# ns1labs/pktvisor

Hardware: AMD Instinct MI355X
Metric: Mpkt/s device-resident (Net+DNS handler parse) (higher is better)
Workload: dtype u8; 1 GPU; C2: Net+DNS handlers, 64 B UDP (Eth+IPv4+UDP+22 B), Zipf IPs, host_spec 10.x.x.x/8; records_per_gpu=10000000, handlers=net v1 + dns v1 (default groups), parallelism=dp1

## Files before the change

### pktvisor_amd/csrc/pv_kernels.hip

```cpp
#include <cstring>
#include <hip/hip_runtime.h>
#include <rocprim/rocprim.hpp>
#include <stdint.h>

#include "pv_layout.h"
#include "pv_geodb.h"

#define PV_BLOCK 256
#define PV_C __attribute__((address_space(4)))
#ifdef PV_STAMPS
#define STAMP_DECL                                                                           \
    uint64_t st_acc[8] = {0, 0, 0, 0, 0, 0, 0, 0};                                          \
    uint64_t st_prev = __builtin_amdgcn_s_memtime();
#define STAMP(k)                                                                             \
    {                                                                                        \
        const uint64_t now = __builtin_amdgcn_s_memtime();                                   \
        st_acc[k] += now - st_prev;                                                          \
        st_prev = now;                                                                       \
    }
#define STAMP_FLUSH                                                                          \
    if ((threadIdx.x & 63) == 0)                                                             \
        for (int k_ = 0; k_ < 8; k_++) P.stamps[((uint64_t)blockIdx.x * (blockDim.x / 64) + threadIdx.x / 64) * 8 + k_] = st_acc[k_];
#else
#define STAMP_DECL
// ... 1628 lines not shown
            const uint64_t m = __ballot(isdns);
            if (m) {
                uint32_t q = 0;
                if (lane == 0) q = atomicAdd(&S.nd, (uint32_t)__popcll(m));
                q = __builtin_amdgcn_readlane(q, 0);
                const uint32_t below = __builtin_amdgcn_mbcnt_hi((uint32_t)(m >> 32), __builtin_amdgcn_mbcnt_lo((uint32_t)m, 0u));
                if (isdns) {
                    PV_G uint4 *dd = reinterpret_cast<PV_G uint4 *>(K.dq) + 2 * (dq_base + q + below);
                    dd[0] = dm.a;
                    dd[1] = dm.b;
                }
            }
            if (tops && i <= r1 && !(K.dbg & 128)) K.iplog[i] = ek;
            if (K.tcp_emit) {
                const uint64_t tm = __ballot(istcp);
                if (tm) {
                    if (lane == 0) K.tmask[t] = tm;
                    tcp_seg_store(K.tseg, K.tseg_cnt, K.tseg_cap, hasseg, seg, lane);
                }
            }
        }
        STAMP(6)
        return released;
    };
    for (uint32_t k = 0; k < ntl; k++) {
        PV_VMCNT((PV_NL_Q - 1) * PV_NL_OPS);
        STAMP(1)
        const uint32_t sl = k % PV_NL_Q, row = k % PV_NL_OROWS;
        const bool rel = tile_body(k, NW.lo[row][lane], __builtin_amdgcn_readfirstlane(NW.lo[row][0]),
                                   tile_of(k) * PV_WT + PV_WT >= n ? (uint32_t)K.rec_bytes : __builtin_amdgcn_readfirstlane(NW.hi[row]),
                                   NW.slot[sl]);
        if (!rel) refill(k);
    }
    PV_VMCNT(0);
    if (wslot != 0xffffffffu) knet_flush(K, wslot, c);
    __syncthreads();
    for (uint32_t b = threadIdx.x; b < PV_HBINS; b += blockDim.x)
        if (S.hist[b]) ksum_add(K, hslot, PV_OFF_PAYLOAD + b, S.hist[b]);
    STAMP_FLUSH
    if (threadIdx.x == 0) {
        P.mq_cnt[blockIdx.x] = 0;
        P.dq_cnt[blockIdx.x] = S.nd;
        if (S.nd) atomicAdd(P.n_dns, S.nd);
    }
}



struct FastRec {
    uint32_t ok, caplen, dir, l4, syn, l4len;
};
struct HostNets {
    uint32_t a0, m0, a1, m1, e0, e1;
};
PV_FN uint32_t hit4(const HostNets &h, uint32_t ip)
{
    const uint32_t m = (((ip ^ h.a0) & h.m0) == 0 ? h.e0 : 0u) | (((ip ^ h.a1) & h.m1) == 0 ? h.e1 : 0u);
    return ip ? m : 0u;
}
PV_FN FastRec fast_fields(const RecW &r, const HostNets &h)
{
    FastRec f;
    f.caplen = r.w[2];
    const uint32_t w3 = r.w[7], w4 = r.w[8], w5 = r.w[9];
    const uint32_t proto = w5 >> 24;
    f.ok = (f.caplen >= 34) & ((w3 & 0xffffffu) == 0x450008u) & (proto != 4) & (proto != 41);
    const uint32_t total = ((w4 & 0xff) << 8) | ((w4 >> 8) & 0xff);
    const uint32_t frag = ((w5 & 0xff) << 8) | ((w5 >> 8) & 0xff);
    const uint32_t l = f.caplen - 14;
    const uint32_t len = (total != 0 && total < l) ? total : l;
    const uint32_t pll = len - 20;
    const bool l4ok = (len > 20) & !(frag & 0x3fff);
    const bool udp = l4ok & (proto == 17) & (pll >= 8);
    const bool tcp = l4ok & (proto == 6) & (pll >= 20);
    f.l4 = udp ? 17u : (tcp ? 6u : 0u);
    f.syn = tcp ? (r.w[15] >> 25) & 1 : 0u;
    f.l4len = pll;
    const uint32_t dst = hit4(h, r.at(46)), src = hit4(h, r.at(42));
    f.dir = dst ? 0u : (src ? 1u : 2u);
    return f;
}
PV_FN uint32_t dns_port_bf(uint32_t pw)
{
    const uint32_t sport = ((pw & 0xff) << 8) | ((pw >> 8) & 0xff);
    const uint32_t dport = ((pw >> 8) & 0xff00) | (pw >> 24);
    const bool dd = (dport == 53) | (dport == 5353) | (dport == 5355) | (dport == 53000);
    const bool sd = (sport == 53) | (sport == 5353) | (sport == 5355) | (sport == 53000);
    return dd ? sport : (sd ? dport : 0u);
}
PV_FN Parsed fast_parsed(const FastRec &f, const RecW &r, uint32_t ts_nano, uint64_t off)
{
    Parsed o;
    o.caplen = f.caplen;
    o.sec = r.w[0];
    o.nsec = ts_nano ? (int32_t)r.w[1] : (int32_t)(r.w[1] * 1000u);
    o.frame = off + 16;
    o.l3 = 4; o.l4 = (uint8_t)f.l4; o.has4 = 1; o.has6 = 0; o.syn = (uint8_t)f.syn; o.dir = (uint8_t)f.dir;
    o.v4 = o.frame + 14; o.v6 = 0;
    o.l4off = f.l4 ? o.frame + 34 : 0;
    o.l4len = f.l4 ? f.l4len : 0;
    return o;
}
__device__ __forceinline__ SlowOut net_slow_p(const PvParams *__restrict__ Pp, const SAcc R, uint64_t off, uint64_t i)
{
    PV_CREF(PvParams) P = *(const PV_C PvParams *)Pp;
    NetK K;
    K.recs = P.recs; K.offs = P.offs; K.n = P.n; K.rec_bytes = P.rec_bytes; K.gbase = P.gbase;
    K.sum = P.sum; K.cpc = P.cpc; K.iplog = P.iplog; K.dq = P.dq; K.flags = P.flags;
    K.n_shift = 0; K.skip_before = 0; K.slot0 = P.slot_of[0];
    K.net_groups = P.net_groups; K.dbg = 0; K.net_filter_all = 0;
    K.n_dshift = P.n_dshift; K.dskip_before = P.dskip_before;
    K.tcp_emit = P.tcp_emit; K.tseg_cap = P.tseg_cap; K.tseg = P.tseg; K.tseg_cnt = P.tseg_cnt; K.tmask = P.tmask;
    K.ndeep_net = nullptr; K.ndeep_dns = nullptr; K.gfilt = nullptr;
    return net_slow_body(R, parse_cfg(P), P, K, off, i, K.slot0, true);
}

#ifndef PV_REG_MINW
#define PV_REG_MINW 2
#endif
struct NetRegState {
    uint32_t hist[PV_HBINS];
    uint32_t nd, nx, ns;
    int64_t dord[PV_MAX_SHIFTS];
};
__device__ __forceinline__ void win_load(const PV_G uint8_t *recs, uint32_t off, uint4 (&W)[5])
{
    const PV_G uint4 *p = reinterpret_cast<const PV_G uint4 *>(recs + (off & ~3u));
#pragma unroll
    for (int j = 0; j < 5; j++) W[j] = p[j];
}
__device__ __forceinline__ void win_words(const uint4 (&W)[5], uint32_t sh, RecW &r)
{
    uint32_t x[17];
#pragma unroll
    for (int k = 0; k < 4; k++) { x[4 * k] = W[k].x; x[4 * k + 1] = W[k].y; x[4 * k + 2] = W[k].z; x[4 * k + 3] = W[k].w; }
    x[16] = W[4].x;
#pragma unroll
    for (int j = 0; j < 16; j++) r.w[j] = __builtin_amdgcn_alignbyte(x[j + 1], x[j], sh);
}
#ifdef PV_TSTAMPS
#define PV_TST_NET ((1u << 20) + (1u << 18))
#define TST_WALL(P, k) if (threadIdx.x == 0) (P).stamps[PV_TST_NET + 4ull * blockIdx.x + (k)] = wall_clock64();
#define TST_WALL_XCC(P) \
    if (threadIdx.x == 0) (P).stamps[PV_TST_NET + 4ull * blockIdx.x] = (wall_clock64() & ~(0xfull << 60)) | (uint64_t)__builtin_amdgcn_s_getreg(20 | (3 << 11)) << 60;
#else
#define TST_WALL_XCC(P)
#define TST_WALL(P, k)
#endif
__device__ __forceinline__ void net_ranges(PV_CREF(PvParams) P, bool contig, uint32_t &lb0, uint32_t &lb1, uint32_t &step)
{
    lb0 = blockIdx.x; lb1 = P.grid_main; step = gridDim.x;
    if (contig) { lb0 = min(blockIdx.x * P.cb_fan, P.grid_main); lb1 = min(lb0 + P.cb_fan, P.grid_main); step = 1; }
}
struct FuseRing {
    struct Sec {
        uint32_t ip[PV_RING_SLOTS][PV_WT];
        uint64_t dm[PV_RING_SLOTS];
    } sec[2];
};
template <uint32_t NW, bool TC = false, bool FUSE = false, bool RING = false>
__device__ __forceinline__ void net_fast_reg(const PvParams *__restrict__ Pp, FuseRing *ring = nullptr)
{
    static_assert(!RING || (FUSE && TC && NW == PV_RING_WAVES), "the ring is the fused kernel's");
    PV_CREF(PvParams) P = *(const PV_C PvParams *)Pp;
    __shared__ NetRegState S;
    TST_WALL_XCC(P)
    const uint32_t wave = __builtin_amdgcn_readfirstlane(threadIdx.x >> 6), lane = threadIdx.x & 63;
    for (uint32_t b = threadIdx.x; b < PV_HBINS; b += (FUSE ? 64u * NW : blockDim.x)) S.hist[b] = 0;
    if (threadIdx.x == 0) { S.nd = 0; S.nx = 0; S.ns = 0; }
    if (threadIdx.x < PV_MAX_SHIFTS) S.dord[threadIdx.x] = P.dpos[threadIdx.x];
    __syncthreads();
    const PV_G uint8_t *const recs = P.recs;
    const bool compact = P.ip_compact;
    const PV_G uint32_t *const offs = P.offs;
    const uint64_t n = P.n, last = n - 1;
    const uint32_t slot = P.slot_of[0];
    const uint32_t groups = P.net_groups;
    const bool tops = groups & PV_NET_TOP_IPS_BIT, card = groups & PV_NET_CARDINALITY_BIT;
    const uint32_t ts_nano = P.ts_nano;
    HostNets h;
    {
        const uint32_t n4 = P.nets.n4;
        h.a0 = P.nets.v4_addr[0]; h.m0 = P.nets.v4_mask[0]; h.e0 = n4 > 0 ? ~0u : 0u;
        h.a1 = P.nets.v4_addr[1]; h.m1 = P.nets.v4_mask[1]; h.e1 = n4 > 1 ? ~0u : 0u;
    }
    const uint64_t nwt = (n + PV_WT - 1) / PV_WT;
    uint64_t cd = 0, cl = 0;
    NetCtr c;
    c.zero();
    bool any = false;
    uint32_t secn = 0;
#ifdef PV_RANGE_AB
    uint32_t lb0, lb1, lbstep;
    net_ranges(P, FUSE || P.net_contig, lb0, lb1, lbstep);
    for (uint32_t lb = lb0; lb < lb1; lb += lbstep) {
#else
    for (uint32_t lb = FUSE ? blockIdx.x * P.cb_fan : blockIdx.x; lb < (FUSE ? min(blockIdx.x * P.cb_fan + P.cb_fan, P.grid_main) : P.grid_main);
         lb += FUSE ? 1u : gridDim.x) {
#endif
    const uint64_t wbeg = (uint64_t)lb * P.wt_per_block;
    const uint64_t wend = min<uint64_t>(wbeg + P.wt_per_block, nwt);
    const uint32_t ntl = wend > wbeg + wave ? (uint32_t)((wend - wbeg - wave + NW - 1) / NW) : 0u;
    any |= ntl != 0;
    const uint32_t nsk = RING ? pv_ring_sections(wend > wbeg ? (uint32_t)(wend - wbeg) : 0u) * PV_RING_K : 0u;
    auto tile_of = [&](uint32_t k) -> uint64_t { return wbeg + wave + (uint64_t)NW * min(k, RING && !ntl ? 0u : ntl - 1); };
    auto off_of = [&](uint32_t k) -> uint32_t { return offs[min<uint64_t>(tile_of(k) * PV_WT + lane, last)]; };
    PV_G uint64_t *const trash = P.trash + ((uint64_t)blockIdx.x * NW + wave) * 256;
    auto tile = [&](uint32_t k, uint32_t off, const uint4 (&W)[5]) {
        const bool live = k < ntl;
        const uint64_t t = tile_of(k);
        const uint64_t r0 = t * PV_WT, i = r0 + lane;
        const bool active = live && i < n;
        RecW rw;
        win_words(W, off & 3, rw);
        const FastRec f = fast_fields(rw, h);
        const bool fast = active & (f.ok != 0);
        const uint64_t slowm = __ballot(active & !fast);
        cd += fast ? 1ull << (f.dir * 16) : 0ull;
        cl += fast ? (1ull << (f.l4 == 17 ? 0u : (f.l4 == 6 ? 16u : 32u))) + ((uint64_t)f.syn << 48) : 0ull;
        uint32_t hv = fast ? f.caplen : PV_NOH;
        const uint32_t ip = f.dir == 0 ? rw.at(42) : rw.at(46);
        const bool ipok = fast & (f.dir != 2) & (ip != 0);
        uint64_t ek = tops && ipok ? ((uint64_t)slot << 60) | ((uint64_t)TM_IPV4 << 56) | ((uint64_t)card << 33) |
                                         ((uint64_t)f.dir << 32) | ip
                                   : 0ull;
        if (card && !tops) {
            if (ipok) {
                uint64_t h1, h2;
                murmur_8((uint64_t)(int64_t)(int32_t)ip, h1, h2);
                __hip_atomic_fetch_min(P.cpc + (uint64_t)slot * PV_MIN_WORDS + (uint64_t)(f.dir == 0 ? CPC_SRC : CPC_DST) * PV_CPC_COUPONS +
                                           cpc_coupon(h1, h2),
                                       (int64_t)(P.gbase + i), __ATOMIC_RELAXED, __HIP_MEMORY_SCOPE_AGENT);
            }
        }
        const uint32_t port = (fast & (f.l4 == 17)) ? dns_port_bf(rw.at(50)) : 0u;
        DnsMsgW dm{};
        bool isdns = port != 0;
        if (__ballot(isdns)) {
            if (isdns) {
                const Parsed o = fast_parsed(f, rw, ts_nano, off);
                uint32_t dp = 0;
                for (uint32_t q = 0; q < P.n_dshift; q++) dp += (int64_t)(4 * i) >= S.dord[q];
                const SAcc R{recs, nullptr, 0, 0, 0, 1};
                DnsMsg d = dns_msg_of(P, R, o, i, port, dp, dp >= P.dskip_before, false);
                d.fkey = fast_flowkey(rw);
                dm = msg_words(d);
            }
        }
        bool istcp = fast & (f.l4 == 6), hasseg = false;
        PvTcpSeg seg;
        const uint32_t temit = P.tcp_emit;
        if (temit && __ballot(istcp)) {
            if (istcp) hasseg = tcp_seg_fast(rw, fast_parsed(f, rw, ts_nano, off), i, seg);
        }
        if (slowm) {
            uint32_t q = 0;
            if (lane == 0) q = atomicAdd(&S.ns, (uint32_t)__popcll(slowm));
            q = __builtin_amdgcn_readlane(q, 0) + __builtin_amdgcn_mbcnt_hi((uint32_t)(slowm >> 32), __builtin_amdgcn_mbcnt_lo((uint32_t)slowm, 0u));
            if (active && !fast) P.slow_list[wbeg * PV_WT + q] = (uint32_t)i;
        }
        if (__ballot(hv != PV_NOH && hv > 65535)) {
            if (hv != PV_NOH && hv > 65535) { atomicOr(P.flags, PVF_BIG_CAPLEN); hv = 65535; }
        }
        hist_add(S.hist, P.sum + (uint64_t)slot * PV_SUM_WORDS + PV_OFF_PAYLOAD, hv, lane);
        const uint64_t m = __ballot(isdns);
        if (m) {
            uint32_t q = 0;
            if (lane == 0) q = atomicAdd(&S.nd, (uint32_t)__popcll(m));
            q = __builtin_amdgcn_readlane(q, 0);
            const uint32_t below = __builtin_amdgcn_mbcnt_hi((uint32_t)(m >> 32), __builtin_amdgcn_mbcnt_lo((uint32_t)m, 0u));
            if (isdns) {
                PV_G uint4 *dd = reinterpret_cast<PV_G uint4 *>(P.dq) + 2 * (wbeg * PV_WT + q + below);
                dd[0] = dm.a;
                dd[1] = dm.b;
            }
        }
        if (TC || tops) {
            if (TC || compact) {
                const bool v4 = ek && ((ek >> 32) & ~1ull) == (P.ip_base >> 32);
                const uint64_t xm = __ballot(active && ek && !v4);
                const uint64_t dbit = __ballot(v4 && ((ek >> 32) & 1));
                if constexpr (RING) {
                    FuseRing::Sec &rs = ring->sec[secn & 1];
                    const uint32_t q = pv_ring_slot(wave, k);
                    rs.ip[q][lane] = active && v4 ? (uint32_t)ek : 0u;
                    if (lane == 0) rs.dm[q] = dbit;
                } else if (TC) {
#ifdef PV_FUSE_NOSTORE
                    if constexpr (!FUSE)
#endif
                    {
                    PV_G uint32_t *const l32 = live ? P.iplog32 + i : reinterpret_cast<PV_G uint32_t *>(trash) + lane;
                    PV_G uint64_t *const ldw = live ? P.ipdir + t : trash + 32;
                    *l32 = active && v4 ? (uint32_t)ek : 0u;
                    *ldw = dbit;
                    }
                } else if (live) {
                    if (active) P.iplog32[i] = v4 ? (uint32_t)ek : 0u;
                    if (lane == 0) P.ipdir[t] = dbit;
                }
                if (xm) {
                    uint32_t q = 0;
                    if (lane == 0) q = atomicAdd(&S.nx, (uint32_t)__popcll(xm));
                    q = __builtin_amdgcn_readlane(q, 0);
                    const uint32_t below = __builtin_amdgcn_mbcnt_hi((uint32_t)(xm >> 32), __builtin_amdgcn_mbcnt_lo((uint32_t)xm, 0u));
                    if (active && ek && !v4) {
                        P.iplog[wbeg * PV_WT + q + below] = ek;
                        P.ipx_rep[wbeg * PV_WT + q + below] = (uint32_t)i;
                    }
                }
            } else if (active) {
                P.iplog[i] = ek;
            }
        }
        if (temit) {
            const uint64_t tm = __ballot(istcp);
            if (tm) {
                if (lane == 0) P.tmask[t] = tm;
                tcp_seg_store(P.tseg, P.tseg_cnt, P.tseg_cap, hasseg, seg, lane);
            }
        }
    };
    static_assert(PV_RING_K == 3, "a section is one turn of the pipeline loop");
    if (RING ? nsk : ntl) {
        uint4 W0[5], W1[5], W2[5];
        uint32_t o0 = off_of(0), o1 = off_of(1), o2 = off_of(2);
        win_load(recs, o0, W0);
        win_load(recs, o1, W1);
        for (uint32_t k = 0; k < (RING ? nsk : ntl); k += 3) {
            const uint32_t oN = off_of(k + 3);
            win_load(recs, o2, W2);
            tile(k, o0, W0);
            const uint32_t oN1 = off_of(k + 4);
            win_load(recs, oN, W0);
            o0 = oN;
            tile(k + 1, o1, W1);
            const uint32_t oN2 = off_of(k + 5);
            win_load(recs, oN1, W1);
            o1 = oN1;
            tile(k + 2, o2, W2);
            o2 = oN2;
            if constexpr (RING) {
                lds_barrier();
                secn++;
            }
        }
    }
    if constexpr (FUSE && !RING) __builtin_amdgcn_s_waitcnt(PV_WAIT_VMCNT0);
    lds_barrier();
    if (threadIdx.x == 0) {
        P.mq_cnt[lb] = 0;
        P.dq_cnt[lb] = S.nd;
        if (compact) P.ipx_cnt[lb] = S.nx;
        P.slow_cnt[lb] = S.ns;
        if (S.nd) atomicAdd(P.n_dns, S.nd);
        if (S.ns) atomicAdd(P.n_slow, S.ns);
        S.nd = 0;
        S.nx = 0;
        S.ns = 0;
    }
    lds_barrier();
    }
    {
        const uint32_t fin = (uint32_t)(cd & 0xffff), fout = (uint32_t)((cd >> 16) & 0xffff), funk = (uint32_t)((cd >> 32) & 0xffff);
        const uint32_t nf = fin + fout + funk;
        c.nev += nf; c.n4 += nf;
        c.nin += fin; c.nout += fout; c.nunk += funk;
        c.nudp += (uint32_t)(cl & 0xffff); c.ntcp += (uint32_t)((cl >> 16) & 0xffff);
        c.noth += (uint32_t)((cl >> 32) & 0xffff); c.nsyn += (uint32_t)(cl >> 48);
    }
    NetK K;
    K.sum = P.sum; K.net_groups = groups; K.net_filter_all = 0; K.gfilt = nullptr;
    if (any) knet_flush(K, slot, c);
    lds_barrier();
    for (uint32_t b = threadIdx.x; b < PV_HBINS; b += (FUSE ? 64u * NW : blockDim.x))
        if (S.hist[b]) ksum_add(K, slot, PV_OFF_PAYLOAD + b, S.hist[b]);
    TST_WALL(P, 1)
}

#ifndef PV_SPAN_MAX
#define PV_SPAN_MAX 6144
#endif
typedef uint32_t v4u32 __attribute__((ext_vector_type(4)));
struct NetSpanState {
    uint32_t hist[PV_HBINS];
    uint32_t nd, ns;
    int64_t dord[PV_MAX_SHIFTS];
    v4u32 buf[4][PV_SPAN_MAX / 16 + 8];
};
struct SpanX {
    v4u32 v0, v1, v2, v3, v4, v5;
};
__device__ __forceinline__ void span_load(const PV_G uint8_t *recs, uint32_t o, uint32_t lane, SpanX &X, uint32_t &b)
{
    const uint32_t o0 = __builtin_amdgcn_readfirstlane(o), o63 = __builtin_amdgcn_readlane(o, 63);
    const uint32_t b16 = o0 & ~15u;
    const uint32_t len = o63 + 80u - b16;
    const PV_G v4u32 *ps = reinterpret_cast<const PV_G v4u32 *>(recs + b16);
    const bool sp = o63 >= o0 && len <= PV_SPAN_MAX && !__ballot(o < o0 || o > o63);
    b = sp ? b16 : 0xffffffffu;
    const uint32_t lim = sp ? len : 0u;
#define PV_SPAN_LD(j) X.v##j = ps[16u * (lane + 64u * j) < lim ? lane + 64u * j : 0u]
    PV_SPAN_LD(0); PV_SPAN_LD(1); PV_SPAN_LD(2); PV_SPAN_LD(3); PV_SPAN_LD(4); PV_SPAN_LD(5);
#undef PV_SPAN_LD
}
extern "C" __global__ void __launch_bounds__(256) __attribute__((amdgpu_waves_per_eu(PV_REG_MINW))) pv_net_kernel_span(const PvParams *__restrict__ Pp)
{
    PV_CREF(PvParams) P = *(const PV_C PvParams *)Pp;
    __shared__ NetSpanState S;
    constexpr uint32_t NW = 4;
    const uint32_t wave = __builtin_amdgcn_readfirstlane(threadIdx.x >> 6), lane = threadIdx.x & 63;
    for (uint32_t b = threadIdx.x; b < PV_HBINS; b += blockDim.x) S.hist[b] = 0;
    if (threadIdx.x == 0) { S.nd = 0; S.ns = 0; }
    if (threadIdx.x < PV_MAX_SHIFTS) S.dord[threadIdx.x] = P.dpos[threadIdx.x];
    __syncthreads();
    const PV_G uint8_t *const recs = P.recs;
    const PV_G uint32_t *const offs = P.offs;
    const uint64_t n = P.n, last = n - 1;
    const uint32_t slot = P.slot_of[0];
    const uint32_t groups = P.net_groups;
    const bool card = groups & PV_NET_CARDINALITY_BIT;
    const uint32_t ts_nano = P.ts_nano;
    HostNets h;
    {
        const uint32_t n4 = P.nets.n4;
        h.a0 = P.nets.v4_addr[0]; h.m0 = P.nets.v4_mask[0]; h.e0 = n4 > 0 ? ~0u : 0u;
        h.a1 = P.nets.v4_addr[1]; h.m1 = P.nets.v4_mask[1]; h.e1 = n4 > 1 ? ~0u : 0u;
    }
    const uint64_t nwt = (n + PV_WT - 1) / PV_WT;
    uint64_t cd = 0, cl = 0;
    v4u32 *Lq = S.buf[wave];
    for (uint32_t lb = blockIdx.x; lb < P.grid_main; lb += gridDim.x) {
    const uint64_t wbeg = (uint64_t)lb * P.wt_per_block;
    const uint64_t wend = min<uint64_t>(wbeg + P.wt_per_block, nwt);
    const uint32_t ntl = wend > wbeg + wave ? (uint32_t)((wend - wbeg - wave + NW - 1) / NW) : 0u;
    auto tile_of = [&](uint32_t k) -> uint64_t { return wbeg + wave + (uint64_t)NW * min(k, ntl - 1); };
    auto off_of = [&](uint32_t k) -> uint32_t { return offs[min<uint64_t>(tile_of(k) * PV_WT + lane, last)]; };
    auto tile = [&](uint32_t k, uint32_t off, const SpanX &X, uint32_t b) {
        const uint64_t t = tile_of(k);
        const uint64_t i = t * PV_WT + lane;
        const bool active = i < n;
        RecW rw;
        if (b != 0xffffffffu) {
            Lq[lane] = X.v0; Lq[lane + 64] = X.v1; Lq[lane + 128] = X.v2;
            Lq[lane + 192] = X.v3; Lq[lane + 256] = X.v4; Lq[lane + 320] = X.v5;
            asm volatile("" ::: "memory");
            const uint32_t rel = off - b;
            const v4u32 *q = Lq + (rel >> 4);
            uint32_t x[24];
#pragma unroll
            for (int j = 0; j < 6; j++) {
                const v4u32 v = q[j];
                x[4 * j] = v.x; x[4 * j + 1] = v.y; x[4 * j + 2] = v.z; x[4 * j + 3] = v.w;
            }
            uint32_t m1 = 0u - ((rel >> 2) & 1), m2 = 0u - ((rel >> 3) & 1);
            asm volatile("" : "+v"(m1), "+v"(m2));
            uint32_t y[19], z[17];
#pragma unroll
            for (int m = 0; m < 19; m++) y[m] = (x[m + 1] & m1) | (x[m] & ~m1);
#pragma unroll
            for (int m = 0; m < 17; m++) z[m] = (y[m + 2] & m2) | (y[m] & ~m2);
#pragma unroll
            for (int j = 0; j < 16; j++) rw.w[j] = __builtin_amdgcn_alignbyte(z[j + 1], z[j], rel & 3);
            asm volatile("" ::: "memory");
        } else {
            uint4 W[5];
            win_load(recs, off, W);
            win_words(W, off & 3, rw);
        }
        const FastRec f = fast_fields(rw, h);
        const bool fast = active & (f.ok != 0);
        cd += fast ? 1ull << (f.dir * 16) : 0ull;
        cl += fast ? (1ull << (f.l4 == 17 ? 0u : (f.l4 == 6 ? 16u : 32u))) + ((uint64_t)f.syn << 48) : 0ull;
        {
            const uint64_t sm = __ballot(active & !fast);
            if (sm) {
                uint32_t q = 0;
                if (lane == 0) q = atomicAdd(&S.ns, (uint32_t)__popcll(sm));
                q = __builtin_amdgcn_readlane(q, 0) + __builtin_amdgcn_mbcnt_hi((uint32_t)(sm >> 32), __builtin_amdgcn_mbcnt_lo((uint32_t)sm, 0u));
                if (active && !fast) P.slow_list[wbeg * PV_WT + q] = (uint32_t)i;
            }
        }
        uint32_t hv = fast ? f.caplen : PV_NOH;
        const uint32_t ip = f.dir == 0 ? rw.at(42) : rw.at(46);
        const bool ipok = fast & (f.dir != 2) & (ip != 0);
        const uint32_t port = (fast & (f.l4 == 17)) ? dns_port_bf(rw.at(50)) : 0u;
        DnsMsgW dm{};
        const bool isdns = port != 0;
        if (__ballot(isdns)) {
            if (isdns) {
                const Parsed o = fast_parsed(f, rw, ts_nano, off);
                uint32_t dp = 0;
                for (uint32_t q = 0; q < P.n_dshift; q++) dp += (int64_t)(4 * i) >= S.dord[q];
                const SAcc R{recs, nullptr, 0, 0, 0, 1};
                DnsMsg dmsg = dns_msg_of(P, R, o, i, port, dp, dp >= P.dskip_before, false);
                dmsg.fkey = fast_flowkey(rw);
                dm = msg_words(dmsg);
            }
        }
        const bool istcp = fast & (f.l4 == 6);
        bool hasseg = false;
        PvTcpSeg seg;
        const uint32_t temit = P.tcp_emit;
        if (temit && __ballot(istcp)) {
            if (istcp) hasseg = tcp_seg_fast(rw, fast_parsed(f, rw, ts_nano, off), i, seg);
        }
        if (__ballot(hv != PV_NOH && hv > 65535)) {
            if (hv != PV_NOH && hv > 65535) { atomicOr(P.flags, PVF_BIG_CAPLEN); hv = 65535; }
        }
        hist_add(S.hist, P.sum + (uint64_t)slot * PV_SUM_WORDS + PV_OFF_PAYLOAD, hv, lane);
        const uint64_t m = __ballot(isdns);
        if (m) {
            uint32_t q = 0;
            if (lane == 0) q = atomicAdd(&S.nd, (uint32_t)__popcll(m));
            q = __builtin_amdgcn_readlane(q, 0);
            const uint32_t below = __builtin_amdgcn_mbcnt_hi((uint32_t)(m >> 32), __builtin_amdgcn_mbcnt_lo((uint32_t)m, 0u));
            if (isdns) {
                PV_G uint4 *dd = reinterpret_cast<PV_G uint4 *>(P.dq) + 2 * (wbeg * PV_WT + q + below);
                dd[0] = dm.a;
                dd[1] = dm.b;
            }
        }
        const uint64_t ek = ipok ? ((uint64_t)card << 33) | ((uint64_t)f.dir << 32) | ip : 0ull;
        P.iplog32[i] = (uint32_t)ek;
        P.ipdir[t] = __ballot(ipok && f.dir == 1);
        if (temit) {
            const uint64_t tm = __ballot(istcp);
// ... 535 lines not shown
        uint64_t cur = cur4[j];
        if (cur == 0) {
            const uint64_t prev = atomicCAS((unsigned long long *)&S.key[b + j], 0ull, (unsigned long long)ck);
            cur = prev == 0 ? ck : prev;
        }
        if (cur == ck) {
            atomicAdd(&S.cnt[b + j], w);
            if (rep < S.rep[b + j]) atomicMin(&S.rep[b + j], rep);
            return true;
        }
    }
    return false;
}
template <class St>
__device__ __forceinline__ void comb_spill(PV_CREF(PvParams) P, St &S, PV_G ulonglong2 *sp, uint64_t ck, uint32_t w,
                                           uint32_t rep)
{
    const ulonglong2 e = comb_entry(ck, w, rep);
    sp[atomicAdd(&S.nsp, 1u)] = e;
    comb_count(P, S, e.x);
}
template <uint32_t CN, class St>
__device__ __forceinline__ void comb_add(PV_CREF(PvParams) P, St &S, PV_G ulonglong2 *sp, uint64_t ck, uint32_t w,
                                         uint32_t rep)
{
    uint32_t pos = (uint32_t)(fmix64(ck) >> 20) & (CN - 1);
#if PV_CB_BUCKET
    for (int g = 0; g < 4; g++)
        if (comb_bucket(P, S, ((pos & ~3u) + 4u * g) & (CN - 1), ck, w, rep)) return;
    comb_spill(P, S, sp, ck, w, rep);
    return;
#endif
    for (int probe = 0; probe < 16; probe++) {
        uint64_t cur = S.key[pos];
        if (cur == 0) {
            const uint64_t prev = atomicCAS((unsigned long long *)&S.key[pos], 0ull, (unsigned long long)ck);
            cur = prev == 0 ? ck : prev;
        }
        if (cur == ck) {
            atomicAdd(&S.cnt[pos], w);
            if (rep < S.rep[pos]) atomicMin(&S.rep[pos], rep);
            return;
        }
        pos = (pos + 1) & (CN - 1);
    }
    comb_spill(P, S, sp, ck, w, rep);
}

template <uint32_t CN, class St>
__device__ __forceinline__ void comb_add_pre(PV_CREF(PvParams) P, St &S, PV_G ulonglong2 *sp, uint64_t ck, uint32_t w,
                                             uint32_t rep, uint32_t pos, uint64_t cur0, uint32_t rep0)
{
    uint64_t cur = cur0;
#if PV_CB_BUCKET
    if (cur == 0) {
        const uint64_t prev = atomicCAS((unsigned long long *)&S.key[pos], 0ull, (unsigned long long)ck);
        cur = prev == 0 ? ck : prev;
        rep0 = 0xffffffffu;
    }
    if (cur == ck) {
        atomicAdd(&S.cnt[pos], w);
        if (rep < rep0) atomicMin(&S.rep[pos], rep);
        return;
    }
    for (int g = 1; g <= 4; g++)
        if (comb_bucket(P, S, ((pos & ~3u) + 4u * g) & (CN - 1), ck, w, rep)) return;
    comb_spill(P, S, sp, ck, w, rep);
    return;
#endif
    for (int probe = 0; probe < 16; probe++) {
        if (probe) { cur = S.key[pos]; rep0 = 0; }
        if (cur == 0) {
            const uint64_t prev = atomicCAS((unsigned long long *)&S.key[pos], 0ull, (unsigned long long)ck);
            cur = prev == 0 ? ck : prev;
            rep0 = 0xffffffffu;
        }
        if (cur == ck) {
            atomicAdd(&S.cnt[pos], w);
            if (rep < rep0 || probe) atomicMin(&S.rep[pos], rep);
            return;
        }
        pos = (pos + 1) & (CN - 1);
    }
    comb_spill(P, S, sp, ck, w, rep);
}

__device__ __forceinline__ uint32_t comb_hash32(uint32_t x)
{
    x ^= x >> 16;
    x *= 0x85ebca6bu;
    x ^= x >> 13;
    x *= 0xc2b2ae35u;
    return x ^ (x >> 16);
}
template <uint32_t CN2>
__device__ __forceinline__ uint32_t comb_cpos(uint32_t ip, uint32_t dir)
{
    return (comb_hash32(ip) & (CN2 - 2u)) | (((uint32_t)__popc(ip) ^ dir) & 1u);
}
template <class St>
__device__ __forceinline__ void comb_chit(St &S, uint32_t pos, uint32_t rel, uint32_t rel0)
{
    const uint32_t sh = 16u * (pos & 1u);
    atomicAdd(&S.ccnt[pos >> 1], 1u << sh);
    if (rel < rel0) {
        uint32_t old = S.crep[pos >> 1];
        while (rel < ((old >> sh) & 0xffffu)) {
            const uint32_t prev = atomicCAS(&S.crep[pos >> 1], old, (old & ~(0xffffu << sh)) | rel << sh);
            if (prev == old) break;
            old = prev;
        }
    }
}
template <class St>
__device__ __forceinline__ bool comb_cbucket(St &S, uint32_t b, uint32_t par, uint32_t ip, uint32_t rel)
{
    const uint4 *kp = reinterpret_cast<const uint4 *>(&S.ckey[b]);
    const uint4 lo = kp[0], hi = kp[1];
    const uint32_t cur4[4] = {par ? lo.y : lo.x, par ? lo.w : lo.z, par ? hi.y : hi.x, par ? hi.w : hi.z};
#pragma unroll
    for (int j = 0; j < 4; j++) {
        const uint32_t s = b + 2u * j + par;
        uint32_t cur = cur4[j];
        if (cur == 0) {
            const uint32_t prev = atomicCAS(&S.ckey[s], 0u, ip);
            cur = prev == 0 ? ip : prev;
        }
        if (cur == ip) {
            comb_chit(S, s, rel, 0xffffffffu);
            return true;
        }
    }
    return false;
}
template <uint32_t CN2, class St>
__device__ __forceinline__ void comb_cadd_pre(PV_CREF(PvParams) P, St &S, PV_G ulonglong2 *sp, uint32_t ip, uint32_t dir,
                                              uint32_t base, uint32_t rel, uint32_t pos, uint32_t cur0, uint32_t rel0)
{
    uint32_t cur = cur0;
    if (cur == 0) {
        const uint32_t prev = atomicCAS(&S.ckey[pos], 0u, ip);
        cur = prev == 0 ? ip : prev;
        rel0 = 0xffffffffu;
    }
    if (cur == ip) {
        comb_chit(S, pos, rel, rel0);
        return;
    }
    for (uint32_t g = 1; g <= 4; g++)
        if (comb_cbucket(S, ((pos & ~7u) + 8u * g) & (CN2 - 1), pos & 1u, ip, rel)) return;
    comb_spill(P, S, sp, P.ip_base | (uint64_t)dir << 32 | ip, 1u, base + rel);
}

__device__ __forceinline__ uint32_t block_excl_scan(uint32_t v, uint32_t *wsum, uint32_t &total)
{
    const uint32_t lane = threadIdx.x & 63, wv = threadIdx.x >> 6, nw = (blockDim.x + 63) >> 6;
    uint32_t incl = v;
#pragma unroll
    for (int o = 1; o < 64; o <<= 1) {
        const uint32_t t = __shfl_up(incl, o, 64);
        if (lane >= (uint32_t)o) incl += t;
    }
    if (lane == 63) wsum[wv] = incl;
    __syncthreads();
    uint32_t base = 0, tot = 0;
    for (uint32_t k = 0; k < nw; k++) {
        const uint32_t s = wsum[k];
        if (k < wv) base += s;
        tot += s;
    }
    __syncthreads();
    total = tot;
    return base + incl - v;
}

template <bool FUSE, class T>
__device__ __forceinline__ T ld_own(const PV_G T *p)
{
    if constexpr (FUSE) return __hip_atomic_load(p, __ATOMIC_RELAXED, __HIP_MEMORY_SCOPE_AGENT);
    else return *p;
}
template <bool RING>
__device__ __forceinline__ FuseRing *fuse_ring()
{
    if constexpr (RING) {
        __shared__ FuseRing r;
        return &r;
    } else
        return nullptr;
}
template <uint32_t CN, class St>
__device__ __forceinline__ void comb_init(St &S, uint32_t nreg, uint32_t tid, uint32_t nt)
{
    for (uint32_t j = tid; j < CN; j += nt) { S.key[j] = 0; S.cnt[j] = 0; S.rep[j] = 0xffffffffu; }
    for (uint32_t r = tid; r < nreg; r += nt) {
        S.h[r] = 0;
        if (!(r & 1)) S.tb[r >> 1] = 0;
    }
    if (tid == 0) S.nsp = 0;
}
template <uint32_t CN, class St>
__device__ __forceinline__ void comb_crange_own(PV_CREF(PvParams) P, St &S, PV_G ulonglong2 *sp, uint32_t gr, uint32_t cbase,
                                                uint32_t tid, uint32_t bd)
{
    const PV_G uint32_t *ip4 = P.iplog32;
    uint64_t a, z;
    wg_records(P, gr, a, z);
    const uint32_t nn = (uint32_t)(z - a), ra = (uint32_t)(a - cbase);
    for (uint32_t j0 = tid; j0 < nn; j0 += PV_CB_U * bd) {
        uint32_t ipv[PV_CB_U];
        uint64_t dw[PV_CB_U];
#pragma unroll
        for (int u = 0; u < PV_CB_U; u++) {
            const uint32_t j = j0 + u * bd;
            ipv[u] = j < nn ? ld_own<true>(ip4 + a + j) : 0u;
            dw[u] = j < nn ? ld_own<true>(P.ipdir + ((a + j) >> 6)) : 0ull;
        }
        uint32_t dir[PV_CB_U], pos[PV_CB_U], cur[PV_CB_U], rp[PV_CB_U];
#pragma unroll
        for (int u = 0; u < PV_CB_U; u++) {
            const uint64_t r = a + j0 + (uint64_t)u * bd;
            dir[u] = (uint32_t)(dw[u] >> (r & 63)) & 1u;
            pos[u] = comb_cpos<2 * CN>(ipv[u], dir[u]);
            cur[u] = ipv[u] ? S.ckey[pos[u]] : 0u;
            rp[u] = ipv[u] ? (S.crep[pos[u] >> 1] >> (16u * (pos[u] & 1u))) & 0xffffu : 0u;
        }
#pragma unroll
        for (int u = 0; u < PV_CB_U; u++)
            if (ipv[u]) comb_cadd_pre<2 * CN>(P, S, sp, ipv[u], dir[u], cbase, ra + j0 + u * bd, pos[u], cur[u], rp[u]);
    }
}
template <uint32_t CN, uint32_t NR, bool FUSE = false, bool RING = false>
__device__ __forceinline__ void topn_combine(PV_CREF(PvParams) P, const PvParams *__restrict__ Pp = nullptr)
{
    using St = CombState<CN, NR>;
    __shared__ St S;
    constexpr uint32_t CK = 16;
    constexpr bool CAN = CN * 2 == CK * PV_CB_THREADS && NR <= 2048;
    bool early = false;
    if constexpr (FUSE) {
        static_assert(sizeof(St) + sizeof(NetRegState) <= 160 * 1024, "pv_net_combine_plain: the Net state and the combine table in one CU's LDS");
        constexpr uint32_t NETW = 4;
        const uint32_t e0 = blockIdx.x * P.cb_fan, e1 = min(e0 + P.cb_fan, P.grid_main);
        uint64_t ea = 0, ez = 0, eb, ey = 0;
        if (e1 > e0) { wg_records(P, e0, ea, ez); wg_records(P, e1 - 1, eb, ey); }
#ifndef PV_FUSE_NO_EARLY
        early = CAN && P.cb_compact && e1 > e0 + 1 && P.ip_compact && (P.net_groups & PV_NET_TOP_IPS_BIT) && blockDim.x == PV_CB_THREADS &&
                ey - ea <= 65535;
#endif
        FuseRing *const ring = fuse_ring<RING>();
        if constexpr (RING) {
            static_assert(CAN && sizeof(St) + sizeof(NetRegState) + sizeof(FuseRing) <= 160 * 1024, "pv_net_combine_ring: the ring beside them");
            static_assert(PV_CB_THREADS == 64 * (NETW + PV_RING_SLOTS), "an inserting thread a slot's lane");
            early = true;
        }
        if (__builtin_amdgcn_readfirstlane(threadIdx.x >> 6) < NETW) {
            net_fast_reg<NETW, true, true, RING>(Pp, ring);
            __builtin_amdgcn_s_waitcnt(PV_WAIT_VMCNT0);
        } else if constexpr (RING) {
            const uint32_t tid = threadIdx.x - 64u * NETW, nt = blockDim.x - 64u * NETW;
            const uint32_t slot = tid >> 6, lane = tid & 63;
            PV_G ulonglong2 *const sp = reinterpret_cast<PV_G ulonglong2 *>(P.tp_buf) + (uint64_t)e0 * P.mq_cap;
            const uint64_t nwt = (P.n + PV_WT - 1) / PV_WT;
            lds_barrier();
            comb_init<CN>(S, 2u << P.reg_log2, tid, nt);
            uint32_t secn = 0;
            for (uint32_t gr = e0; gr < e1; gr++) {
                const uint64_t wbeg = (uint64_t)gr * P.wt_per_block, wend = min<uint64_t>(wbeg + P.wt_per_block, nwt);
                const uint32_t ns = pv_ring_sections(wend > wbeg ? (uint32_t)(wend - wbeg) : 0u);
                const uint32_t ra = (uint32_t)(wbeg * PV_WT - ea);
                for (uint32_t s = 0; s < ns; s++, secn++) {
                    lds_barrier();
                    const FuseRing::Sec &rs = ring->sec[secn & 1];
                    const uint32_t ip = rs.ip[slot][lane];
                    if (ip) {
                        const uint32_t dir = (uint32_t)(rs.dm[slot] >> lane) & 1u, pos = comb_cpos<2 * CN>(ip, dir);
                        comb_cadd_pre<2 * CN>(P, S, sp, ip, dir, (uint32_t)ea, ra + (pv_ring_tile(s, slot) * PV_WT + lane), pos, S.ckey[pos],
                                              (S.crep[pos >> 1] >> (16u * (pos & 1u))) & 0xffffu);
                    }
                }
                lds_barrier();
                lds_barrier();
            }
            lds_barrier();
        } else {
            const uint32_t tid = threadIdx.x - 64u * NETW, nt = blockDim.x - 64u * NETW;
            lds_barrier();
            comb_init<CN>(S, 2u << P.reg_log2, tid, nt);
            for (uint32_t gr = e0; gr < e1; gr++) {
                lds_barrier();
                lds_barrier();
                if (early && gr + 1 < e1)
                    comb_crange_own<CN>(P, S, reinterpret_cast<PV_G ulonglong2 *>(P.tp_buf) + (uint64_t)e0 * P.mq_cap, gr, (uint32_t)ea, tid, nt);
            }
            lds_barrier();
        }
        __syncthreads();
        TST_WALL(P, 2)
    }
    if constexpr (!FUSE) {
        if (P.plain_chain && (*P.n_dns | *P.n_slow)) return;
    }
    TST_DECL
    const uint32_t nreg = 2u << P.reg_log2;
    const uint32_t g0 = blockIdx.x * P.cb_fan, g1 = min(g0 + P.cb_fan, P.grid_main);
    if constexpr (FUSE) {
        uint32_t bad = 0;
        for (uint32_t gr = g0; gr < g1; gr++) bad |= ld_own<true>(P.dq_cnt + gr) | ld_own<true>(P.slow_cnt + gr);
        if (bad) return;
    }
    const uint64_t wbase = (uint64_t)g0 * P.mq_cap;
    PV_G ulonglong2 *sp = reinterpret_cast<PV_G ulonglong2 *>(P.tp_buf) + wbase;
    PV_G ulonglong2 *out = reinterpret_cast<PV_G ulonglong2 *>(P.cb) + wbase;
    uint32_t cbase = 0;
    uint32_t other = 1;
    if constexpr (CAN) {
        if (P.cb_compact && (RING || g1 - g0 > 1) && P.ip_compact && (P.net_groups & PV_NET_TOP_IPS_BIT) && blockDim.x == PV_CB_THREADS) {
            uint64_t a0, z0, a1, z1;
            wg_records(P, g0, a0, z0);
            wg_records(P, g1 - 1, a1, z1);
            other = z1 - a0 > 65535 ? 1u : 0u;
            for (uint32_t gr = g0; gr < g1; gr++) other |= ld_own<FUSE>(P.mq_cnt + gr) | ld_own<FUSE>(P.ipx_cnt + gr);
            cbase = (uint32_t)a0;
        }
    }
    if constexpr (!FUSE) {
    for (uint32_t j = threadIdx.x; j < CN; j += blockDim.x) { S.key[j] = 0; S.cnt[j] = 0; S.rep[j] = 0xffffffffu; }
    for (uint32_t r = threadIdx.x; r < nreg; r += blockDim.x) {
        S.h[r] = 0;
        if (!(r & 1)) S.tb[r >> 1] = 0;
    }
    if (threadIdx.x == 0) S.nsp = 0;
    }
    const bool compact = RING || (CAN && __builtin_amdgcn_readfirstlane(other) == 0);
    if constexpr (!FUSE) __syncthreads();
    TST(0)
    if (compact) {
        if constexpr (CAN) {
            const PV_G uint32_t *ip4 = P.iplog32;
            for (uint32_t gr = RING ? g1 : (FUSE && early ? g1 - 1 : g0); gr < g1; gr++) {
                uint64_t a, z;
                wg_records(P, gr, a, z);
                const uint32_t nn = (uint32_t)(z - a), bd = blockDim.x, ra = (uint32_t)(a - cbase);
                for (uint32_t j0 = threadIdx.x; j0 < nn; j0 += PV_CB_U * bd) {
                    uint32_t ipv[PV_CB_U];
                    uint64_t dw[PV_CB_U];
#pragma unroll
                    for (int u = 0; u < PV_CB_U; u++) {
                        const uint32_t j = j0 + u * bd;
                        ipv[u] = j < nn ? ld_own<FUSE>(ip4 + a + j) : 0u;
                        dw[u] = j < nn ? ld_own<FUSE>(P.ipdir + ((a + j) >> 6)) : 0ull;
                    }
                    uint32_t dir[PV_CB_U], pos[PV_CB_U], cur[PV_CB_U], rp[PV_CB_U];
#pragma unroll
                    for (int u = 0; u < PV_CB_U; u++) {
                        const uint64_t r = a + j0 + (uint64_t)u * bd;
                        dir[u] = (uint32_t)(dw[u] >> (r & 63)) & 1u;
                        pos[u] = comb_cpos<2 * CN>(ipv[u], dir[u]);
                        cur[u] = ipv[u] ? S.ckey[pos[u]] : 0u;
                        rp[u] = ipv[u] ? (S.crep[pos[u] >> 1] >> (16u * (pos[u] & 1u))) & 0xffffu : 0u;
                    }
#pragma unroll
                    for (int u = 0; u < PV_CB_U; u++)
                        if (ipv[u]) comb_cadd_pre<2 * CN>(P, S, sp, ipv[u], dir[u], cbase, ra + j0 + u * bd, pos[u], cur[u], rp[u]);
                }
            }
        }
    } else
    for (uint32_t gr = g0; gr < g1; gr++) {
    const uint32_t cnt = ld_own<FUSE>(P.mq_cnt + gr);
    const PV_G uint64_t *q = P.mq + (uint64_t)gr * P.mq_cap * 2;
    batched<8>(cnt, [&](uint64_t j) { return PV_E16(q)[j]; },
               [&](uint64_t, ulonglong2 e) { comb_add<CN>(P, S, sp, e.x, (uint32_t)e.y, (uint32_t)(e.y >> 32)); });
    if (P.net_groups & PV_NET_TOP_IPS_BIT) {
        uint64_t a, z;
        wg_records(P, gr, a, z);
        const PV_G uint64_t *ipl = P.iplog + a;
        if (P.ip_compact) {
            const PV_G uint32_t *ip4 = P.iplog32;
            const uint64_t nn = z - a, bd = blockDim.x;
            const uint64_t ipb = P.ip_base;
            for (uint64_t j0 = threadIdx.x; j0 < nn; j0 += (uint64_t)PV_CB_U * bd) {
                uint32_t ipv[PV_CB_U];
                uint64_t dw[PV_CB_U];
#pragma unroll
                for (int u = 0; u < PV_CB_U; u++) {
                    const uint64_t j = j0 + (uint64_t)u * bd;
                    ipv[u] = j < nn ? ld_own<FUSE>(ip4 + a + j) : 0u;
                    dw[u] = j < nn ? ld_own<FUSE>(P.ipdir + ((a + j) >> 6)) : 0ull;
                }
                uint64_t ck[PV_CB_U], cur[PV_CB_U];
                uint32_t pos[PV_CB_U], rp[PV_CB_U];
#pragma unroll
                for (int u = 0; u < PV_CB_U; u++) {
                    const uint64_t r = a + j0 + (uint64_t)u * bd;
                    ck[u] = ipb | ((dw[u] >> (r & 63)) & 1) << 32 | ipv[u];
                    pos[u] = (uint32_t)(fmix64(ck[u]) >> 20) & (CN - 1);
                    cur[u] = ipv[u] ? S.key[pos[u]] : 0ull;
                    rp[u] = ipv[u] ? S.rep[pos[u]] : 0u;
                }
#pragma unroll
                for (int u = 0; u < PV_CB_U; u++)
                    if (ipv[u]) comb_add_pre<CN>(P, S, sp, ck[u], 1u, (uint32_t)(a + j0 + (uint64_t)u * bd), pos[u], cur[u], rp[u]);
            }
            const uint32_t nx = ld_own<FUSE>(P.ipx_cnt + gr);
            for (uint32_t q = threadIdx.x; q < nx; q += blockDim.x)
                comb_add<CN>(P, S, sp, ld_own<FUSE>(ipl + q), 1u, ld_own<FUSE>(P.ipx_rep + a + q));
        } else {
            batched<PV_CB_U>(z - a, [&](uint64_t j) { return ipl[j]; }, [&](uint64_t j, uint64_t e) {
                if (e) comb_add<CN>(P, S, sp, e, 1u, (uint32_t)(a + j));
            });
        }
    }
    }
    if (threadIdx.x == 0) S.hm = 0;
    __syncthreads();
    TST(1)
    uint32_t rk[CK / 2] = {};
    if (compact) {
        if constexpr (CAN) {
            const uint64_t tk = P.ip_base & (0xffull << 56);
#pragma unroll
            for (uint32_t k = 0; k < CK; k++) {
                const uint32_t ip = S.ckey[threadIdx.x + k * PV_CB_THREADS];
                const uint32_t r = ip ? comb_count(P, S, tk | ip) : 0u;
                rk[k / 2] = k & 1 ? rk[k / 2] | r << 16 : r;
            }
        }
    } else
    for (uint32_t j = threadIdx.x; j < CN; j += blockDim.x)
        if (S.key[j]) comb_count(P, S, comb_entry(S.key[j], S.cnt[j], S.rep[j]).x);
    __syncthreads();
    TST(2)
    const uint32_t per = (nreg + blockDim.x - 1) / blockDim.x;
    const uint32_t r0 = min(threadIdx.x * per, nreg), r1 = min(r0 + per, nreg);
    uint32_t s = 0;
    for (uint32_t r = r0; r < r1; r++) s += S.h[r];
    {
        const uint32_t hb = s ? 1u << (r0 >> P.reg_log2) : 0u;
        const uint64_t b0 = __ballot(hb & 1), b1 = __ballot(hb & 2);
        if ((threadIdx.x & 63) == 0 && (b0 | b1)) atomicOr(&S.hm, (b0 ? 1u : 0u) | (b1 ? 2u : 0u));
    }
    uint32_t total;
    uint32_t run = block_excl_scan(s, S.wsum, total);
    const uint32_t hm = S.hm;
    if (threadIdx.x < 2 && ((hm >> threadIdx.x) & 1)) atomicOr(P.tp_hands, 1u << threadIdx.x);
    if (threadIdx.x == 0) P.cb_hm[blockIdx.x] = hm;
    const uint32_t ng8 = (P.cb_grid + 7) / 8;
    PV_G uint64_t *col = P.cb_run + (blockIdx.x % 8) * ng8 + blockIdx.x / 8;
    for (uint32_t r = r0; r < r1; r++) {
        const uint32_t c = S.h[r];
        if ((hm >> (r >> P.reg_log2)) & 1) col[(uint64_t)r * 8 * ng8] = pv_run_word(run, c, (S.tb[r >> 1] >> (16u * (r & 1u))) & 0xffffu);
        S.h[r] = run;
        run += c;
    }
    lds_barrier();
    TST(3)
    if (compact) {
        if constexpr (CAN) {
#pragma unroll 1
            for (uint32_t q = 0; q < PV_CB_OSWEEP; q++)
#pragma unroll
            for (uint32_t k = 0; k < CK; k++) {
                const uint32_t j = threadIdx.x + k * PV_CB_THREADS, sh = 16u * (j & 1u);
                const uint32_t ip = S.ckey[j];
                if (!ip) continue;
                if (PV_CB_OSWEEP > 1 && ((((rk[k / 2] >> (16u * (k & 1u))) & 0xffffu) * PV_CB_OSWEEP) >> P.reg_log2) != q) continue;
                const uint64_t ck = P.ip_base | (uint64_t)((j ^ (uint32_t)__popc(ip)) & 1u) << 32 | ip;
                const ulonglong2 e = comb_entry(ck, (S.ccnt[j >> 1] >> sh) & 0xffffu, cbase + ((S.crep[j >> 1] >> sh) & 0xffffu));
                out[atomicAdd(&S.h[(rk[k / 2] >> (16u * (k & 1u))) & 0xffffu], 1u)] = e;
            }
        }
    } else
    for (uint32_t j = threadIdx.x; j < CN; j += blockDim.x)
        if (S.key[j]) {
            const ulonglong2 e = comb_entry(S.key[j], S.cnt[j], S.rep[j]);
            out[atomicAdd(&S.h[run_key(P, e.x)], 1u)] = e;
        }
    const uint32_t nsp = S.nsp;
    batched<8>(nsp, [&](uint64_t j) { return sp[j]; },
               [&](uint64_t, ulonglong2 e) { out[atomicAdd(&S.h[run_key(P, e.x)], 1u)] = e; });
    if (threadIdx.x == 0) P.cb_cnt[blockIdx.x] = total;
#ifdef PV_TSTAMPS
    __syncthreads();
#endif
    TST(4)
    TST_FLUSH(0)
    if constexpr (FUSE) { TST_WALL(P, 3) }
}
#ifndef PV_CB_CN
#define PV_CB_CN 8192
#endif
static_assert(PV_SLOTS == 16, "pv_topn_combine folds a table bit to 16 bits a region");
extern "C" __global__ void __launch_bounds__(PV_CB_THREADS) pv_topn_combine(const PvParams *__restrict__ Pp)
{
    PV_CREF(PvParams) P = *(const PV_C PvParams *)Pp;
    topn_combine<PV_CB_CN, 2048>(P);
}
extern "C" __global__ void __launch_bounds__(PV_CB_THREADS) pv_net_combine_plain(const PvParams *__restrict__ Pp)
{
    PV_CREF(PvParams) P = *(const PV_C PvParams *)Pp;
    topn_combine<PV_CB_CN, 2048, true>(P, Pp);
}
extern "C" __global__ void __launch_bounds__(PV_CB_THREADS) pv_net_combine_ring(const PvParams *__restrict__ Pp)
{
    PV_CREF(PvParams) P = *(const PV_C PvParams *)Pp;
    topn_combine<PV_CB_CN, 2048, true, true>(P, Pp);
}
extern "C" __global__ void __launch_bounds__(256) pv_net_iplog(const PvParams *__restrict__ Pp)
{
    PV_CREF(PvParams) P = *(const PV_C PvParams *)Pp;
    const uint32_t wave = __builtin_amdgcn_readfirstlane(threadIdx.x >> 6), lane = threadIdx.x & 63;
    const uint64_t n = P.n, nwt = (n + PV_WT - 1) / PV_WT;
    HostNets h;
    {
        const uint32_t n4 = P.nets.n4;
        h.a0 = P.nets.v4_addr[0]; h.m0 = P.nets.v4_mask[0]; h.e0 = n4 > 0 ? ~0u : 0u;
        h.a1 = P.nets.v4_addr[1]; h.m1 = P.nets.v4_mask[1]; h.e1 = n4 > 1 ? ~0u : 0u;
    }
    for (uint64_t t = (uint64_t)blockIdx.x * 4 + wave; t < nwt; t += (uint64_t)gridDim.x * 4) {
        const uint64_t i = t * PV_WT + lane;
        const uint32_t off = P.offs[min<uint64_t>(i, n - 1)];
        uint4 W[5];
        win_load(P.recs, off, W);
        RecW rw;
        win_words(W, off & 3, rw);
        const FastRec f = fast_fields(rw, h);
        const uint32_t ip = f.dir == 0 ? rw.at(42) : rw.at(46);
        const bool ipok = i < n && f.ok != 0 && f.dir != 2 && ip != 0;
        const uint64_t dbit = __ballot(ipok && f.dir == 1);
        P.iplog32[i] = ipok ? ip : 0u;
        if (lane == 0) P.ipdir[t] = dbit;
    }
}
extern "C" __global__ void __launch_bounds__(PV_CB_THREADS) pv_topn_combine_r12(const PvParams *__restrict__ Pp)
{
    PV_CREF(PvParams) P = *(const PV_C PvParams *)Pp;
    topn_combine<2048, 2u << PV_MAX_REGIONS_LOG2>(P);
}

#define PV_MG_THREADS 512
#ifndef PV_MG_U2
#define PV_MG_U2 4
#endif
#ifndef PV_MG_SEEN
#define PV_MG_SEEN 1
#endif
#define PV_MG_NN 640
#define PV_CREATED (1ull << 63)
#define PV_MV4 (1ull << 62)
#define PV_MN1 (0xffffffull << 32)
#define PV_DL0 (0xffffffffull << 32)
__device__ __forceinline__ bool mv4_key(uint64_t k) { return PV_KEY_METRIC(k) == TM_IPV4 && !((k >> 40) & 1); }
__device__ __forceinline__ uint64_t mv4_norm(uint64_t w) { return w & ~(PV_CREATED | ((w & PV_MV4) ? PV_MN1 : 0ull)); }
struct MergeState {
    alignas(16) uint64_t key[PV_RS];
    uint64_t dl[PV_RS];
    uint32_t nrep[PV_MG_NN];
    uint16_t nidx[PV_MG_NN];
    uint32_t nnew, nbase, ncr;
    uint32_t ip4c;
};
struct MergeRuns {
    uint32_t start[PV_MAX_GRID + 8];
    uint32_t pref[PV_MAX_GRID + 9];
    uint16_t list[PV_MAX_GRID + 8];
    uint32_t wsum[16];
    uint32_t tabs;
};
static_assert(2 * PV_MG_THREADS >= (PV_MAX_GRID + 7) / 8 * 8, "two runs per merge thread");
static_assert(sizeof(MergeState) + sizeof(MergeRuns) <= 80 * 1024, "pv_topn_merge: two workgroups per CU");
extern "C" uint32_t pv_topn_merge_threads() { return PV_MG_THREADS; }
extern "C" __global__ void __launch_bounds__(PV_MG_THREADS) __attribute__((amdgpu_waves_per_eu(4))) pv_topn_merge(const PvParams *__restrict__ Pp)
{
    PV_CREF(PvParams) P = *(const PV_C PvParams *)Pp;
    const uint32_t rk = blockIdx.x;
    const uint32_t r = rk & ((1u << P.reg_log2) - 1);
    const uint32_t hd = rk >> P.reg_log2;
    if (P.plain_chain && (*P.n_dns | *P.n_slow)) return;
    if (!((*P.tp_hands >> hd) & 1)) return;
    if (P.xmerge && (r < P.x_lo || r >= P.x_hi)) return;
    __shared__ MergeRuns U;
    __shared__ MergeState S;
    TST_DECL
    const uint32_t ng8 = (P.cb_grid + 7) / 8, ng = 8 * ng8;
    const uint64_t lcap = (uint64_t)P.cb_fan * P.mq_cap;
    const uint32_t rsl = P.tcap_log2 - P.reg_log2;
    const uint32_t rs = 1u << rsl;
    const uint32_t tbg = hd ? PV_SLOTS + P.dslot_of[0] : P.slot_of[0];
    const uint64_t rbg = ((uint64_t)tbg << P.tcap_log2) + ((uint64_t)r << rsl);
    const bool pf = rs == PV_RS;
    if (pf) {
        static_assert(PV_RS * 8 == 32 * 1024 && PV_MG_THREADS == 512, "four pieces per wave");
        const uint32_t wv = threadIdx.x >> 6, ln = threadIdx.x & 63;
#pragma unroll
        for (int q = 0; q < 4; q++) {
            const uint32_t pc = wv * 4 + q;
// ... 1866 lines not shown
```

Baseline: 31080 Mpkt/s.

## Use LDS-only barriers and workgroup-aggregated counters in the fused ring tail

In the fused ring kernel, the tail phase now uses LDS-only barriers instead of full __syncthreads, which drops the implied wait on outstanding global memory ops. Explicit vmcnt waits are moved to the producer waves. Net counters are summed per wave into LDS and flushed once per workgroup instead of being flushed per wave with global atomics. A bad flag kept in LDS replaces re-reading the per-group dq/slow/mq/ipx counts from global memory. The risk is memory-ordering bugs if some global write is still pending when an LDS-only barrier is crossed.

```diff
diff --git a/pktvisor_amd/csrc/pv_kernels.hip b/pktvisor_amd/csrc/pv_kernels.hip
--- a/pktvisor_amd/csrc/pv_kernels.hip
+++ b/pktvisor_amd/csrc/pv_kernels.hip
@@ -1804,12 +1804,27 @@
     lb0 = blockIdx.x; lb1 = P.grid_main; step = gridDim.x;
     if (contig) { lb0 = min(blockIdx.x * P.cb_fan, P.grid_main); lb1 = min(lb0 + P.cb_fan, P.grid_main); step = 1; }
 }
+#define PV_RING_CTRS 12
 struct FuseRing {
     struct Sec {
         uint32_t ip[PV_RING_SLOTS][PV_WT];
         uint64_t dm[PV_RING_SLOTS];
     } sec[2];
+    uint32_t ctr[PV_RING_CTRS];
+    uint32_t bad;
+    uint32_t pad;
 };
+#ifdef PV_RING_SYNC_TAIL
+#define PV_RING_LDS_TAIL false
+#else
+#define PV_RING_LDS_TAIL true
+#endif
+template <bool LDS>
+__device__ __forceinline__ void tail_barrier()
+{
+    if constexpr (LDS) lds_barrier();
+    else __syncthreads();
+}
 template <uint32_t NW, bool TC = false, bool FUSE = false, bool RING = false>
 __device__ __forceinline__ void net_fast_reg(const PvParams *__restrict__ Pp, FuseRing *ring = nullptr)
 {
@@ -1821,6 +1836,10 @@
     for (uint32_t b = threadIdx.x; b < PV_HBINS; b += (FUSE ? 64u * NW : blockDim.x)) S.hist[b] = 0;
     if (threadIdx.x == 0) { S.nd = 0; S.nx = 0; S.ns = 0; }
     if (threadIdx.x < PV_MAX_SHIFTS) S.dord[threadIdx.x] = P.dpos[threadIdx.x];
+    if constexpr (RING) {
+        if (threadIdx.x < PV_RING_CTRS) ring->ctr[threadIdx.x] = 0;
+        if (threadIdx.x == 0) ring->bad = 0;
+    }
     __syncthreads();
     const PV_G uint8_t *const recs = P.recs;
     const bool compact = P.ip_compact;
@@ -1998,7 +2017,11 @@
             }
         }
     }
+#ifdef PV_RING_NO_RANGE_WAIT
     if constexpr (FUSE && !RING) __builtin_amdgcn_s_waitcnt(PV_WAIT_VMCNT0);
+#else
+    if constexpr (FUSE && (!RING || PV_RING_LDS_TAIL)) __builtin_amdgcn_s_waitcnt(PV_WAIT_VMCNT0);
+#endif
     lds_barrier();
     if (threadIdx.x == 0) {
         P.mq_cnt[lb] = 0;
@@ -2007,6 +2030,7 @@
         P.slow_cnt[lb] = S.ns;
         if (S.nd) atomicAdd(P.n_dns, S.nd);
         if (S.ns) atomicAdd(P.n_slow, S.ns);
+        if constexpr (RING) ring->bad |= S.nd | S.ns;
         S.nd = 0;
         S.nx = 0;
         S.ns = 0;
@@ -2023,8 +2047,34 @@
     }
     NetK K;
     K.sum = P.sum; K.net_groups = groups; K.net_filter_all = 0; K.gfilt = nullptr;
-    if (any) knet_flush(K, slot, c);
+#if defined(PV_RING_NOFLUSH)
+    constexpr bool FLUSH = !RING, WGFLUSH = false;
+#elif defined(PV_RING_WAVE_FLUSH)
+    constexpr bool FLUSH = true, WGFLUSH = false;
+#else
+    constexpr bool FLUSH = true, WGFLUSH = RING;
+#endif
+    if constexpr (WGFLUSH) {
+        static_assert(NC_TOTAL + 1 == PV_RING_CTRS && NC_FILTERED == PV_RING_CTRS, "the counter words, contiguous");
+        auto put = [&](uint32_t w, uint32_t v) {
+            const uint32_t t = wave_sum(v);
+            if (lane == 0 && t) atomicAdd(&ring->ctr[w], t);
+        };
+        put(NC_EVENTS, c.nev); put(NC_SAMPLES, c.nev); put(NC_TOTAL, c.nev - c.nfilt); put(NC_IN, c.nin);
+        put(NC_OUT, c.nout); put(NC_UNK, c.nunk); put(NC_V4, c.n4); put(NC_V6, c.n6);
+        put(NC_UDP, c.nudp); put(NC_TCP, c.ntcp); put(NC_SYN, c.nsyn); put(NC_OTHER, c.noth);
+    } else if constexpr (FLUSH) {
+        if (any) knet_flush(K, slot, c);
+    }
     lds_barrier();
+    if constexpr (WGFLUSH) {
+        if (threadIdx.x < PV_RING_CTRS) {
+            const uint32_t t = ring->ctr[threadIdx.x];
+            if (t && (threadIdx.x == NC_EVENTS || threadIdx.x == NC_SAMPLES || (groups & PV_NET_COUNTERS_BIT)))
+                ksum_add(K, slot, PV_OFF_NET + threadIdx.x, t);
+        }
+    }
+    if constexpr (FLUSH)
     for (uint32_t b = threadIdx.x; b < PV_HBINS; b += (FUSE ? 64u * NW : blockDim.x))
         if (S.hist[b]) ksum_add(K, slot, PV_OFF_PAYLOAD + b, S.hist[b]);
     TST_WALL(P, 1)
@@ -2866,6 +2916,7 @@
     comb_spill(P, S, sp, P.ip_base | (uint64_t)dir << 32 | ip, 1u, base + rel);
 }
 
+template <bool LDS = false>
 __device__ __forceinline__ uint32_t block_excl_scan(uint32_t v, uint32_t *wsum, uint32_t &total)
 {
     const uint32_t lane = threadIdx.x & 63, wv = threadIdx.x >> 6, nw = (blockDim.x + 63) >> 6;
@@ -2876,14 +2927,14 @@
         if (lane >= (uint32_t)o) incl += t;
     }
     if (lane == 63) wsum[wv] = incl;
-    __syncthreads();
+    tail_barrier<LDS>();
     uint32_t base = 0, tot = 0;
     for (uint32_t k = 0; k < nw; k++) {
         const uint32_t s = wsum[k];
         if (k < wv) base += s;
         tot += s;
     }
-    __syncthreads();
+    tail_barrier<LDS>();
     total = tot;
     return base + incl - v;
 }
@@ -2970,7 +3021,7 @@
         }
         if (__builtin_amdgcn_readfirstlane(threadIdx.x >> 6) < NETW) {
             net_fast_reg<NETW, true, true, RING>(Pp, ring);
-            __builtin_amdgcn_s_waitcnt(PV_WAIT_VMCNT0);
+            if constexpr (!(RING && PV_RING_LDS_TAIL)) __builtin_amdgcn_s_waitcnt(PV_WAIT_VMCNT0);
         } else if constexpr (RING) {
             const uint32_t tid = threadIdx.x - 64u * NETW, nt = blockDim.x - 64u * NETW;
             const uint32_t slot = tid >> 6, lane = tid & 63;
@@ -2996,6 +3047,7 @@
                 lds_barrier();
                 lds_barrier();
             }
+            __builtin_amdgcn_s_waitcnt(PV_WAIT_VMCNT0);
             lds_barrier();
         } else {
             const uint32_t tid = threadIdx.x - 64u * NETW, nt = blockDim.x - 64u * NETW;
@@ -3009,9 +3061,10 @@
             }
             lds_barrier();
         }
-        __syncthreads();
+        tail_barrier<RING && PV_RING_LDS_TAIL>();
         TST_WALL(P, 2)
     }
+    constexpr bool LT = RING && PV_RING_LDS_TAIL;
     if constexpr (!FUSE) {
         if (P.plain_chain && (*P.n_dns | *P.n_slow)) return;
     }
@@ -3020,6 +3073,8 @@
     const uint32_t g0 = blockIdx.x * P.cb_fan, g1 = min(g0 + P.cb_fan, P.grid_main);
     if constexpr (FUSE) {
         uint32_t bad = 0;
+        if constexpr (LT) bad = fuse_ring<RING>()->bad;
+        else
         for (uint32_t gr = g0; gr < g1; gr++) bad |= ld_own<true>(P.dq_cnt + gr) | ld_own<true>(P.slow_cnt + gr);
         if (bad) return;
     }
@@ -3034,6 +3089,7 @@
             wg_records(P, g0, a0, z0);
             wg_records(P, g1 - 1, a1, z1);
             other = z1 - a0 > 65535 ? 1u : 0u;
+            if constexpr (!LT)
             for (uint32_t gr = g0; gr < g1; gr++) other |= ld_own<FUSE>(P.mq_cnt + gr) | ld_own<FUSE>(P.ipx_cnt + gr);
             cbase = (uint32_t)a0;
         }
@@ -3128,7 +3184,7 @@
     }
     }
     if (threadIdx.x == 0) S.hm = 0;
-    __syncthreads();
+    tail_barrier<LT>();
     TST(1)
     uint32_t rk[CK / 2] = {};
     if (compact) {
@@ -3144,7 +3200,7 @@
     } else
     for (uint32_t j = threadIdx.x; j < CN; j += blockDim.x)
         if (S.key[j]) comb_count(P, S, comb_entry(S.key[j], S.cnt[j], S.rep[j]).x);
-    __syncthreads();
+    tail_barrier<LT>();
     TST(2)
     const uint32_t per = (nreg + blockDim.x - 1) / blockDim.x;
     const uint32_t r0 = min(threadIdx.x * per, nreg), r1 = min(r0 + per, nreg);
@@ -3156,7 +3212,7 @@
         if ((threadIdx.x & 63) == 0 && (b0 | b1)) atomicOr(&S.hm, (b0 ? 1u : 0u) | (b1 ? 2u : 0u));
     }
     uint32_t total;
-    uint32_t run = block_excl_scan(s, S.wsum, total);
+    uint32_t run = block_excl_scan<LT>(s, S.wsum, total);
     const uint32_t hm = S.hm;
     if (threadIdx.x < 2 && ((hm >> threadIdx.x) & 1)) atomicOr(P.tp_hands, 1u << threadIdx.x);
     if (threadIdx.x == 0) P.cb_hm[blockIdx.x] = hm;
```

Result: faster. 34450 Mpkt/s, median of 6 (+10.8%).
